# shichaoy/pop_up_slam

Measured on AMD Instinct MI355X. Metric: graph-solve iters/sec + final chi2, 1k-pose/5k-edge plane graph, higher is better.
Workload: dtype f64; 1 GPU; C2 synthetic corridor: 1000 SE3 poses, 200 planes, 5000 plane edges, 999 odometry edges (BASELINE.json configs[1], seed 42); jacobian_mode=numeric, total_lm_solves=805

## Files before the change

pop_up_slam_amd/csrc/pps_api.cpp:

```cpp
#include "pps_graph.h"

using namespace pps;
using namespace pps_impl;

namespace pps {
Switches read_switches() {
  auto on = [](const char* k) { return getenv(k) != nullptr; };
  auto num = [](const char* k, long long dflt) { const char* e = getenv(k); return e && *e ? atoll(e) : dflt; };
  Switches s;
  s.k1_thread_form = on("PPS_K1_THREAD_FORM");
  {
    long long plain = num("PPS_PLAIN_SCHEDULE", 0);
    if (on("PPS_PLAIN_SCHEDULE") && plain <= 0) plain = 15;
    s.no_preassemble = (plain & 1) != 0; s.no_solve_flow = (plain & 2) != 0; s.no_root_fuse = (plain & 4) != 0; s.split_expand = (plain & 8) != 0;
  }
  s.no_spec_lin = on("PPS_NO_SPEC_LIN");
  s.no_dual = on("PPS_NO_DUAL");
  s.no_strip = on("PPS_NO_STRIP");
  s.no_incremental = on("PPS_NO_INCREMENTAL");
  s.no_incr_compact = on("PPS_NO_INCR_COMPACT");
  s.verify_upload = on("PPS_DEBUG_VERIFY_UPLOAD");
  s.multi_levels = on("PPS_MULTI_LEVELS");
  s.multi_thread_form = on("PPS_MULTI_THREAD_FORM");
  s.debug_drop_flag = (int)num("PPS_DEBUG_DROP_FLAG", 0);
  if (on("PPS_DEBUG_DROP_FLAG") && s.debug_drop_flag < 1) s.debug_drop_flag = 1;
  s.trace = (int)num("PPS_TRACE", 0);
  if (on("PPS_TRACE") && s.trace < 1) s.trace = 1;
  {
    long long tm = num("PPS_TIMING", 0);
// ... 108 lines not shown
    std::vector<std::pair<std::string, double>> v(g->up_laps.begin(), g->up_laps.end());
    std::sort(v.begin(), v.end());
    for (auto& kv : v) fprintf(stderr, "[upload] %-34s %9.3f ms total\n", kv.first.c_str(), 1e3 * kv.second);
  }
  if (g->acache) analysis_cache_free(g->acache);
  if (g->dev_ready) {
    (void)hipSetDevice(g->props.device);
    (void)hipStreamSynchronize(g->stream);
    free_device(g);
    release_arenas(g);
    if (g->host_result) (void)hipHostFree(g->host_result);
    if (g->ev[0]) (void)hipEventDestroy(g->ev[0]);
    if (g->ev[1]) (void)hipEventDestroy(g->ev[1]);
    for (hipEvent_t e : g->k1_events) (void)hipEventDestroy(e);
    for (hipEvent_t e : g->fk_events) (void)hipEventDestroy(e);
    if (g->d_lms) (void)hipFree(g->d_lms);
    if (g->h_lms) (void)hipHostFree(g->h_lms);
    if (g->d_queries) (void)hipHostFree(g->d_queries);
    if (g->d_results) (void)hipHostFree(g->d_results);
    if (g->d_lm_planes) (void)hipFree(g->d_lm_planes);
    if (g->rp_pin) (void)hipHostFree(g->rp_pin);
    cov_release(g);
    (void)hipStreamDestroy(g->stream);
  }
  delete g;
  return PPS_OK;
}

int pps_get_props(const pps_graph* g, pps_props* out) {
  if (!g || !out) return PPS_EINVAL;
// ... 441 lines not shown
```

pop_up_slam_amd/csrc/pps_device.h:

```cpp
#pragma once

#include <hip/hip_runtime.h>

#include <cstdint>

#include "pps_cost.h"

namespace pps {

struct DevGraph {
  int n_pose = 0, n_plane = 0, pose_ld = 0, plane_ld = 0;
  double *pose_est = nullptr, *pose_lin = nullptr;
  double *plane_est = nullptr, *plane_lin = nullptr;
  int *pose_voff = nullptr, *plane_voff = nullptr;
  int n_obs = 0, n_odo = 0, n_pp = 0, n_lp = 0;
  int obs_ld = 0, odo_ld = 0, pp_ld = 0, lp_ld = 0;
  int *obs_pose = nullptr, *obs_plane = nullptr; double *obs_meas = nullptr, *obs_w = nullptr;
  int n_obs_fixed = 0; double* obs_ray = nullptr;
  int *odo_a = nullptr, *odo_b = nullptr;         double *odo_meas = nullptr, *odo_w = nullptr;
  int *pp_pose = nullptr;                          double *pp_meas = nullptr, *pp_w = nullptr;
  int *lp_plane = nullptr;                         double *lp_meas = nullptr, *lp_w = nullptr;
  double* J = nullptr;
  int64_t joff_obs = 0, joff_odo = 0, joff_pp = 0, joff_lp = 0;
  double* P = nullptr;
// ... 44 lines not shown
  int no_strip = 0;
  unsigned sw = 0;
  double step_ac[4] = {0, 0, 0, 0};
  double* gwork = nullptr;
  int64_t gwork_stride = 0;
};

constexpr double kStatusInternal = 64.0;
enum : unsigned { SW_K1_THREAD_FORM = 1u, SW_NO_SOLVE_FLOW = 2u, SW_NO_ROOT_FUSE = 4u, SW_DEBUG_DROP_FLAG = 8u, SW_DEBUG_DROP_XFLAG = 16u };
struct Switches {
  bool k1_thread_form = false;
  bool no_preassemble = false;
  bool no_solve_flow = false;
  bool no_root_fuse = false;
  bool split_expand = false;
  bool no_spec_lin = false;
  bool no_dual = false;
  bool no_strip = false;
  bool no_incremental = false;
  bool no_incr_compact = false;
  bool verify_upload = false;
  bool multi_levels = false, multi_thread_form = false;
  int debug_drop_flag = 0;
  int trace = 0;
  bool analysis_timing = false, upload_timing = false;
  int multi_timing = 0;
  int multi_split = 0;
  long long multi_thread_factors = 120000;
  unsigned dev_bits() const {
    return (k1_thread_form ? SW_K1_THREAD_FORM : 0u) | (no_solve_flow ? SW_NO_SOLVE_FLOW : 0u) | (no_root_fuse ? SW_NO_ROOT_FUSE : 0u) |
// ... 29 lines not shown
hipError_t step_constants(double ac[4]);
hipError_t launch_linearize(const DevGraph& d, int mode, bool at_estimate, hipStream_t st, const LinGuard* guard = nullptr, hipEvent_t ev0 = nullptr,
                            hipEvent_t ev1 = nullptr);
hipError_t launch_hblocks(const DevGraph& d, hipStream_t st, const LinGuard* guard = nullptr, bool products = true);
bool k1_lane_form(const DevGraph& d, int mode);
bool k1_products(const DevGraph& d, int mode);
hipError_t launch_factor_level(const DevGraph& d, int level_begin, int level_count, int level_max_front, double lambda,
                               hipStream_t st);
hipError_t launch_backsolve_level(const DevGraph& d, int level_begin, int level_count, hipStream_t st);
struct DualAlt {
  double *L, *U, *delta, *result_dev, *chi2_partials, *dn_partials;
  unsigned int* ticket;
  double lambda;
};
hipError_t launch_band_all(const DevGraph& d, const DualAlt* alt, int n_groups, int nwaves_factor, int nwaves_solve, int max_front, int max_panel,
                           int max_group_fronts, double lambda, int epoch, hipStream_t st, hipEvent_t ev0 = nullptr, hipEvent_t ev1 = nullptr);
int band_all_solve_waves(int max_panel, int max_group_fronts);
hipError_t launch_band_factor(const DevGraph& d, int grp_begin, int grp_count, int nwaves, int max_front, double lambda, hipStream_t st,
                              hipEvent_t ev0 = nullptr, hipEvent_t ev1 = nullptr, bool pre = false);
hipError_t launch_band_solve(const DevGraph& d, int grp_begin, int grp_count, int nwaves, int max_panel, int max_group_fronts, hipStream_t st,
                             const DualAlt* alt = nullptr);
hipError_t launch_band_factor_dual(const DevGraph& d, const DualAlt& alt, int grp_begin, int grp_count, int nwaves, int max_front, double lambda,
                                   hipStream_t st, hipEvent_t ev0 = nullptr, hipEvent_t ev1 = nullptr, bool pre = false);
bool band_root_fusable(const DevGraph& d, int grp_count, int max_front);
hipError_t launch_band_root(const DevGraph& d, const DualAlt* alt, int grp, int nwaves_factor, int nwaves_solve, int max_front, int max_panel,
                            int max_group_fronts, double lambda, hipStream_t st, hipEvent_t ev0 = nullptr, hipEvent_t ev1 = nullptr,
                            bool pre = false);
hipError_t launch_trial_dual(const DevGraph& d, const DualAlt& alt, const double* base_pose, const double* base_plane, double* out_pose0,
                             double* out_plane0, double* out_pose1, double* out_plane1, double* host_result0, double seq0, double* host_result1,
                             double seq1, hipStream_t st, int n_trials = 2);
hipError_t launch_trial_lin(const DevGraph& d, const DualAlt& alt, const SpecLin& sl, const double* base_pose, const double* base_plane, double* out_pose0,
                            double* out_plane0, double* out_pose1, double* out_plane1, double* host_result0, double seq0, double* host_result1,
// ... 93 lines not shown
```

pop_up_slam_amd/csrc/pps_graph.h:

```cpp
#pragma once
#include <hip/hip_runtime.h>

#include <algorithm>
#include <charconv>
#include <chrono>
#include <cmath>
#include <cstdio>
#include <cstdlib>
#include <cstring>
#include <mutex>
#include <new>
#include <string>
#include <unordered_map>
#include <vector>

#include "../../include/pps.h"
#include "pps_cov.h"
#include "pps_device.h"
#include "pps_geom.h"
#include "pps_lm.h"
#include "pps_popup_dev.h"
#include "pps_symbolic.h"

namespace pps_impl {
// ... 86 lines not shown
  bool pin_holds_est = false;
  std::unordered_map<std::string, double> up_laps;
  struct UpPatch { size_t off, len; bool exact8 = false; };
  std::vector<UpPatch> up_patches;
  char* patch_host = nullptr; size_t patch_cap = 0;
  size_t up_bytes_sent = 0, up_bytes_total = 0;
  double* host_result = nullptr;
  double seq = 0.0;
  double *spec_pose = nullptr, *spec_plane = nullptr, *spec_chi2_partials = nullptr, *spec_dn_partials = nullptr;
  unsigned int* spec_ticket = nullptr;
  double seq2 = 0.0;
  double *spec_L = nullptr, *spec_U = nullptr, *spec_delta = nullptr;
  double* spec_result = nullptr;
  double *spec_J = nullptr, *spec_P = nullptr, *spec_H = nullptr, *spec_Hf = nullptr;
  bool k3_all = false;
  int k3_nw_factor = 0, k3_nw_solve = 0, k3_max_front = 0, k3_max_panel = 0, k3_max_grp = 0, k3_epoch = 0;
  double *snap_pose = nullptr, *snap_plane = nullptr;
  int snap_version = -1, upload_version = 0;
  int k2t_version = -1;
  int profiling = 0;
  hipEvent_t ev[2] = {nullptr, nullptr};
  unsigned long long launches0 = 0;
  std::vector<char> k1_skip;
  std::vector<hipEvent_t> k1_events;
  std::vector<hipEvent_t> fk_events;
  int fk_used = 0;
  int k1_used = 0;
  float frames_invK[9] = {1, 0, 0, 0, 1, 0, 0, 0, 1};
  std::vector<int> fr_pose;
  std::vector<int> fr_seg_off{0};
  std::vector<float> fr_seg;
  std::vector<int> fr_item_frame, fr_item_plane, fr_item_fid;
  bool frames_dirty = true;
  std::vector<int> fr_slot, fr_pslot;
  long n_removals = 0, fr_cache_removals = -1;
  int fr_hint_version = -2; size_t fr_hint_cursor = 0, fr_hint_items = 0, fr_hint_frames = 0;
  int frames_version = -1;
  int *d_item_frame = nullptr, *d_item_plane = nullptr, *d_item_slot = nullptr, *d_frame_pose_slot = nullptr, *d_frame_seg_off = nullptr;
  float* d_fr_seg = nullptr;
  bool dev_meas_newer = false;
  int n_obs_fixed = 0;
// ... 219 lines not shown
```

pop_up_slam_amd/csrc/pps_k3.hip:

```cpp
#include <algorithm>
#include <atomic>
#include <cstdlib>

#include <hip/hip_ext.h>

#include "pps_kcommon.h"
#include "pps_regtile.h"
#include "pps_front_reg.h"

namespace pps {


constexpr int kLdsLimitBytes = 160 * 1024 - 1024;

int lds_front_limit() {
  int fa = 1;
  while ((size_t)(fa + 1) * ((fa + 1) | 1) * 8 <= (size_t)kLdsLimitBytes) fa++;
  return fa - 1;
}

template <bool USE_LDS>
__global__ __launch_bounds__(256) void k_front_factor(DevGraph d, int level_begin, double lambda) {
  extern __shared__ double lds[];
  const int s = d.level_fronts[level_begin + blockIdx.x];
// ... 417 lines not shown
  __builtin_amdgcn_wave_barrier();
}
struct XGroup { int* flag; int epoch; };
__device__ __forceinline__ void xg_post(const XGroup& x, int s) {
  __builtin_amdgcn_fence(__ATOMIC_RELEASE, "agent");
  if ((threadIdx.x & 63) == 0) __hip_atomic_store(x.flag + s, x.epoch, __ATOMIC_RELAXED, __HIP_MEMORY_SCOPE_AGENT);
}
__device__ __forceinline__ void xg_wait(const DevGraph& d, const XGroup& x, int s) {
  int spin = 0;
  while (__hip_atomic_load(x.flag + s, __ATOMIC_RELAXED, __HIP_MEMORY_SCOPE_AGENT) != x.epoch) {
    if (++spin >= (1 << 21)) { if ((threadIdx.x & 63) == 0) raise_status(&d.result_dev[2], kStatusInternal); break; }
    __builtin_amdgcn_s_sleep(2);
  }
  __builtin_amdgcn_fence(__ATOMIC_ACQUIRE, "agent");
}
template <bool XG = false>
__device__ __forceinline__ void front_extend_add(const DevGraph& d, int rec, int crv0, int lane, double* __restrict__ F, int tr, const XGroup* xg = nullptr) {
  const int cr0 = __builtin_amdgcn_readlane(rec, 5), nch = __builtin_amdgcn_readlane(rec, 6);
  for (int cb = 0; cb < nch; cb += 8) {
    const int crv = cb == 0 ? crv0 : ((lane < 8 * (nch - cb)) ? d.crec[(size_t)(cr0 + cb) * 8 + lane] : 0);
    auto child = [&](int cj, int& n, const double* __restrict__& Uc, const int* __restrict__& tgc) {
      n = __builtin_amdgcn_readlane(crv, 8 * cj);
      const long long uo = ((long long)__builtin_amdgcn_readlane(crv, 8 * cj + 2) << 32) | (unsigned int)__builtin_amdgcn_readlane(crv, 8 * cj + 1);
      const long long eo = ((long long)__builtin_amdgcn_readlane(crv, 8 * cj + 4) << 32) | (unsigned int)__builtin_amdgcn_readlane(crv, 8 * cj + 3);
      Uc = d.U + uo; tgc = d.ea_tgt + eo;
    };
    int cj = 0;
    for (; cj < 8 && cb + cj < nch; cj++) {
      int n; const double* Uc; const int* tgc;
      child(cj, n, Uc, tgc);
// ... 65 lines not shown
#ifndef PPS_NO_FMA
#pragma clang fp contract(fast)
#endif
    if (!SCALED) solve_pivot_scale(lk, dinv);
#define PPS_BS(U) case U: tj -= lk[U] * row_bcast_d<U>(tj); [[fallthrough]];
    switch (p < 16 ? p - 1 : 15) {
      PPS_BS(15) PPS_BS(14) PPS_BS(13) PPS_BS(12) PPS_BS(11) PPS_BS(10) PPS_BS(9) PPS_BS(8)
      PPS_BS(7) PPS_BS(6) PPS_BS(5) PPS_BS(4) PPS_BS(3) PPS_BS(2)
      case 1: tj -= lk[1] * row_bcast_d<1>(tj); [[fallthrough]];
      default: break;
    }
#undef PPS_BS
    tj *= dinv;
}

template <bool GROUP = true, bool TR = false, bool XG = false>
__device__ __forceinline__ void wave_front_solve(const DevGraph& d, int rec, double* __restrict__ W, double* __restrict__ X, int slot, int* flow = nullptr, const XGroup* xg = nullptr) {
  const int lane = threadIdx.x & 63;
  const int s = __builtin_amdgcn_readlane(rec, 0);
  (void)s;
  if (TR) PPS_TR(0);
  const int p = __builtin_amdgcn_readlane(rec, 1), b = __builtin_amdgcn_readlane(rec, 2), f = p + b;
  const double* __restrict__ Lp = d.L + (((long long)__builtin_amdgcn_readlane(rec, 10) << 32) | (unsigned int)__builtin_amdgcn_readlane(rec, 9));
  const int pslot = GROUP ? __builtin_amdgcn_readlane(rec, 14) : -1;
  const int* __restrict__ ix = b == 0 ? d.frec : (pslot >= 0 ? d.cmap + __builtin_amdgcn_readlane(rec, 15) : d.bidx + __builtin_amdgcn_readlane(rec, 8));
  double* xb = W;
  double* PL = W + kBandMaxRows;
  const int ix0r = ix[lane < b ? lane : 0], ix1r = ix[lane + 64 < b ? lane + 64 : 0];
  const int pix = d.pidx[__builtin_amdgcn_readlane(rec, 7) + (lane < p ? lane : 0)];
  const int n = (f + 1) * p;
  double tj = 0.0, dinv = 0.0;
// ... 9 lines not shown
    double lbv[12];
#pragma unroll
    for (int u = 0; u < 12; u++) { const int i = part + 4 * u; lbv[u] = LB[(i < b ? i : blast) * p]; }
#pragma unroll
    for (int u = 0; u < 16; u++) { const double l = Lp[(u < p ? u : p - 1) * p + lc]; lk[u] = lane < u ? l : 0.0; }
    const double dg = Lp[lc * p + lc], yr = Lp[f * p + jc];
    const int ix0 = lane < b ? ix0r : 0, ix1 = lane + 64 < b ? ix1r : 0;
    double g0 = 0.0, g1 = 0.0;
    const int xpar = XG ? __builtin_amdgcn_readlane(rec, 13) : -1;
    if (pslot < 0 && xpar < 0) { g0 = d.delta[ix0]; g1 = d.delta[ix1]; }
    if (flow) { dinv = 1.0 / dg; solve_pivot_scale(lk, dinv); }
    if (pslot >= 0) {
      if (flow) flow_wait(d, flow, pslot);
      const double* __restrict__ Xp = X + (size_t)pslot * kBandMaxRows; g0 = Xp[ix0]; g1 = Xp[ix1];
    } else if (XG && xpar >= 0) {
      xg_wait(d, *xg, xpar);
      g0 = d.delta[ix0]; g1 = d.delta[ix1];
    }
    if (TR) PPS_TR(1);
    if (lane < b) xb[lane] = g0;
    if (lane + 64 < b) xb[lane + 64] = g1;
    __builtin_amdgcn_wave_barrier();
    if (TR) PPS_TR(2);
    if (!flow) dinv = 1.0 / dg;
    double a[4] = {part == 0 ? yr : 0.0, 0.0, 0.0, 0.0};
#pragma unroll
    for (int u = 0; u < 12; u++) { const int i = part + 4 * u; const double x = i < b ? xb[i] : 0.0; a[u & 3] -= lbv[u] * x; }
    for (int i0 = 48; i0 < b; i0 += 48) {
#pragma unroll
      for (int u = 0; u < 12; u++) { const int i = i0 + part + 4 * u; lbv[u] = LB[(i < b ? i : blast) * p]; }
#pragma unroll
// ... 51 lines not shown
    if (pre32) {
      const int sh = p <= 16 ? 4 : 5, np = 64 >> sh;
      const int j = lane & ((1 << sh) - 1), part = lane >> sh;
      const int jc = j < p ? j : 0;
      const int blast = b > 0 ? b - 1 : 0;
#pragma unroll
      for (int u = 0; u < 12; u++) { const int i = part + np * u; lbq[u] = PL[(p + (i < b ? i : blast)) * p + jc]; }
      yq = PL[f * p + jc];
    }
  }
  if (pslot >= 0) {
    if (flow) flow_wait(d, flow, pslot);
    const double* __restrict__ Xp = X + (size_t)pslot * kBandMaxRows;
    g0 = Xp[ix0]; g1 = Xp[ix1];
  } else if (XG && xpar >= 0) {
    xg_wait(d, *xg, xpar);
    g0 = d.delta[ix0]; g1 = d.delta[ix1];
  }
  if (lane < b) xb[lane] = g0;
  if (lane + 64 < b) xb[lane + 64] = g1;
  __builtin_amdgcn_wave_barrier();
  if (TR) PPS_TR(2);
  {
#ifndef PPS_NO_FMA
#pragma clang fp contract(fast)
#endif
    if (!flow) {
#pragma unroll
      for (int u = 0; u < 16; u++) { const int k = k0 + u; const double l = PL[(k < p ? k : p - 1) * p + lc]; lk[u] = lane < k ? l : 0.0; }
      dinv = 1.0 / PL[lc * p + lc];
    }
// ... 35 lines not shown
    }
    solve_pivot_chain(p, lk, dinv, tj);
  }
  if (TR) PPS_TR(4);
  if (lane < p) d.delta[pix] = tj;
  if (TR) PPS_TR(5);
  if (!GROUP) return;
  double* __restrict__ Xs = X + (size_t)slot * kBandMaxRows;
  if (lane < p) Xs[lane] = tj;
  if (lane < b) Xs[p + lane] = g0;
  if (lane + 64 < b) Xs[p + lane + 64] = g1;
  if (flow) flow_post(d, flow, slot, pslot < 0);
  if (XG) { if (__builtin_amdgcn_readlane(rec, 6) > 0) xg_post(*xg, s); }
}

template <bool TR = false, bool XG = false>
__device__ __forceinline__ void body_band_solve_flow(const DevGraph& d, int g, int lds_doubles_per_wave, double* __restrict__ lds, int mg, const XGroup* xg = nullptr) {
  const int wave = uni(threadIdx.x >> 6), nw = blockDim.x >> 6;
  double* W = lds + (size_t)wave * lds_doubles_per_wave;
  double* X = lds + (size_t)nw * lds_doubles_per_wave;
  int* flow = reinterpret_cast<int*>(X + (size_t)mg * kBandMaxRows);
  const int2 span = reinterpret_cast<const int2*>(d.grp_span)[4 * (size_t)g];
  const int g0 = uni(span.x), gn = uni(span.y);
  const int i_first = g0 + gn - 1 - wave;
  int rec = i_first >= g0 ? d.frec[(size_t)i_first * 16 + (threadIdx.x & 15)] : 0;
  for (int q = threadIdx.x; q < gn; q += blockDim.x) flow[q] = 0;
  __syncthreads();
  for (int i = i_first; i >= g0; i -= nw) {
    wave_front_solve<true, TR, XG>(d, rec, W, X, i - g0, flow, xg);
    if (i - nw >= g0) rec = d.frec[(size_t)(i - nw) * 16 + (threadIdx.x & 15)];
  }
}
template <bool TR = false>
__device__ __forceinline__ void body_band_solve(const DevGraph& d, int g, int lds_doubles_per_wave, double* __restrict__ lds) {
  const int wave = uni(threadIdx.x >> 6), nw = blockDim.x >> 6;
  double* W = lds + (size_t)wave * lds_doubles_per_wave;
  double* X = lds + (size_t)nw * lds_doubles_per_wave;
  const int l0 = uni(d.grp_lvl_off[g]), l1 = uni(d.grp_lvl_off[g + 1]);
  int off[5], r4[4];
  {
    const int4 ga = reinterpret_cast<const int4*>(d.grp_span)[2 * (size_t)g], gb = reinterpret_cast<const int4*>(d.grp_span)[2 * (size_t)g + 1];
    off[0] = uni(ga.x); off[1] = uni(ga.w); off[2] = uni(gb.x); off[3] = uni(gb.y); off[4] = uni(gb.z);
  }
  const int g0 = off[0];
// ... 135 lines not shown
}

__global__ __launch_bounds__(512) void k_band_factor_all(DevGraph d, DualAlt alt, double lambda, int lds_doubles_per_wave, int epoch) {
  extern __shared__ double lds[];
  XGroup xg{d.k3_flag, epoch};
  if (blockIdx.y) { d.L = alt.L; d.U = alt.U; d.delta = alt.delta; d.result_dev = alt.result_dev; lambda = alt.lambda; xg.flag += d.n_fronts; }
  body_band_factor_pre<true>(d, blockIdx.x, lambda, lds_doubles_per_wave, lds, &xg);
}
__global__ __launch_bounds__(768) void k_band_solve_all(DevGraph d, DualAlt alt, int n_groups, int lds_doubles_per_wave, int mg, int epoch) {
  extern __shared__ double lds[];
  XGroup xg{d.k3_flag + 2 * d.n_fronts, epoch};
  if (blockIdx.y) { d.L = alt.L; d.U = alt.U; d.delta = alt.delta; d.result_dev = alt.result_dev; xg.flag += d.n_fronts; }
  body_band_solve_flow<false, true>(d, n_groups - 1 - (int)blockIdx.x, lds_doubles_per_wave, lds, mg, &xg);
}

__global__ __launch_bounds__(512) void k_band_factor_pre(DevGraph d, DualAlt alt, int grp_begin, double lambda, int lds_doubles_per_wave) {
  extern __shared__ double lds[];
  if (blockIdx.y) { d.L = alt.L; d.U = alt.U; d.delta = alt.delta; d.result_dev = alt.result_dev; lambda = alt.lambda; }
  body_band_factor_pre(d, grp_begin + blockIdx.x, lambda, lds_doubles_per_wave, lds);
}

__global__ __launch_bounds__(512) void k_band_factor_lean_trace(DevGraph d, DualAlt alt, int grp_begin, double lambda, int lds_doubles_per_wave) {
  extern __shared__ double lds[];
  body_band_factor<true, false, true>(d, grp_begin + blockIdx.x, lambda, lds_doubles_per_wave, lds);
}

__global__ __launch_bounds__(256) __attribute__((amdgpu_waves_per_eu(1, 1)))
void k_band_factor_r5(DevGraph d, DualAlt alt, int grp_begin, double lambda, int lds_doubles_per_wave) {
  extern __shared__ double lds[];
  if (blockIdx.y) { d.L = alt.L; d.U = alt.U; d.delta = alt.delta; d.result_dev = alt.result_dev; lambda = alt.lambda; }
// ... 9 lines not shown
    hipError_t e = hipFuncSetAttribute(reinterpret_cast<const void*>(&k_band_factor<false>), hipFuncAttributeMaxDynamicSharedMemorySize, kLdsLimitBytes);
    if (e == hipSuccess) e = hipFuncSetAttribute(reinterpret_cast<const void*>(&k_band_factor<true>), hipFuncAttributeMaxDynamicSharedMemorySize, kLdsLimitBytes);
    if (e == hipSuccess) e = hipFuncSetAttribute(reinterpret_cast<const void*>(&k_band_solve), hipFuncAttributeMaxDynamicSharedMemorySize, kLdsLimitBytes);
    if (e == hipSuccess) e = hipFuncSetAttribute(reinterpret_cast<const void*>(&k_band_solve_trace), hipFuncAttributeMaxDynamicSharedMemorySize, kLdsLimitBytes);
    if (e == hipSuccess) e = hipFuncSetAttribute(reinterpret_cast<const void*>(&k_band_solve_flow), hipFuncAttributeMaxDynamicSharedMemorySize, kLdsLimitBytes);
    if (e == hipSuccess) e = hipFuncSetAttribute(reinterpret_cast<const void*>(&k_band_factor_pre), hipFuncAttributeMaxDynamicSharedMemorySize, kLdsLimitBytes);
    if (e == hipSuccess) e = hipFuncSetAttribute(reinterpret_cast<const void*>(&k_band_solve_flow_trace), hipFuncAttributeMaxDynamicSharedMemorySize, kLdsLimitBytes);
    if (e == hipSuccess) e = hipFuncSetAttribute(reinterpret_cast<const void*>(&k_band_factor_r5), hipFuncAttributeMaxDynamicSharedMemorySize, kLdsLimitBytes);
    if (e == hipSuccess) e = hipFuncSetAttribute(reinterpret_cast<const void*>(&k_band_factor_lean_trace), hipFuncAttributeMaxDynamicSharedMemorySize, kLdsLimitBytes);
    if (e == hipSuccess) e = hipFuncSetAttribute(reinterpret_cast<const void*>(&k_band_root<false, false>), hipFuncAttributeMaxDynamicSharedMemorySize, kLdsLimitBytes);
    if (e == hipSuccess) e = hipFuncSetAttribute(reinterpret_cast<const void*>(&k_band_root<true, false>), hipFuncAttributeMaxDynamicSharedMemorySize, kLdsLimitBytes);
    if (e == hipSuccess) e = hipFuncSetAttribute(reinterpret_cast<const void*>(&k_band_root<false, true>), hipFuncAttributeMaxDynamicSharedMemorySize, kLdsLimitBytes);
    if (e == hipSuccess) e = hipFuncSetAttribute(reinterpret_cast<const void*>(&k_band_root<true, true>), hipFuncAttributeMaxDynamicSharedMemorySize, kLdsLimitBytes);
    if (e == hipSuccess) e = hipFuncSetAttribute(reinterpret_cast<const void*>(&k_band_factor_all), hipFuncAttributeMaxDynamicSharedMemorySize, kLdsLimitBytes);
    if (e == hipSuccess) e = hipFuncSetAttribute(reinterpret_cast<const void*>(&k_band_solve_all), hipFuncAttributeMaxDynamicSharedMemorySize, kLdsLimitBytes);
    if (e != hipSuccess) return e;
    g_band_attr_set[dev & 63] = true;
  }
  return hipSuccess;
}

static hipError_t launch_band_factor_impl(const DevGraph& d, const DualAlt& alt, int ny, int grp_begin, int grp_count, int nwaves, int max_front, double lambda,
                                          hipStream_t st, hipEvent_t ev0 = nullptr, hipEvent_t ev1 = nullptr, bool pre = false) {
  if (grp_count == 0) return hipSuccess;
  { const hipError_t e = ensure_band_attrs(); if (e != hipSuccess) return e; }
  const bool reg_only = max_front + 1 <= kRegRows && !(ny == 2 && d.trace != nullptr);
  const int per_wave = (int)(band_lds_bytes(max_front, reg_only) / sizeof(double));
  const size_t bytes = (size_t)per_wave * nwaves * sizeof(double);
  if (reg_only && d.trace != nullptr)
    PPS_LAUNCH(k_band_factor_lean_trace, dim3(grp_count, ny), dim3(64 * nwaves), bytes, st, d, alt, grp_begin, lambda, per_wave);
// ... 61 lines not shown
    const int want = nwaves_factor > (max_group_fronts < 8 ? max_group_fronts : 8) ? nwaves_factor : (max_group_fronts < 8 ? max_group_fronts : 8);
    if ((size_t)pws * want * sizeof(double) + flow_fixed <= (size_t)kLdsLimitBytes) nw = want; else flow = false;
  }
  const size_t bf = (size_t)pwf * nw * sizeof(double);
  const size_t bs = flow ? (size_t)pws * nw * sizeof(double) + flow_fixed : ((size_t)pws * nw + (size_t)max_group_fronts * kBandMaxRows) * sizeof(double);
  const size_t bytes = bf > bs ? bf : bs;
  const DualAlt a2 = alt ? *alt : DualAlt{};
  if (pre && flow) PPS_LAUNCH_EV(ev0, ev1, (k_band_root<true, true>), dim3(1, alt ? 2 : 1), dim3(64 * nw), bytes, st, d, a2, grp, lambda, pwf, pws, max_group_fronts);
  else if (pre) PPS_LAUNCH_EV(ev0, ev1, (k_band_root<true, false>), dim3(1, alt ? 2 : 1), dim3(64 * nw), bytes, st, d, a2, grp, lambda, pwf, pws, max_group_fronts);
  else if (flow) PPS_LAUNCH_EV(ev0, ev1, (k_band_root<false, true>), dim3(1, alt ? 2 : 1), dim3(64 * nw), bytes, st, d, a2, grp, lambda, pwf, pws, max_group_fronts);
  else PPS_LAUNCH_EV(ev0, ev1, (k_band_root<false, false>), dim3(1, alt ? 2 : 1), dim3(64 * nw), bytes, st, d, a2, grp, lambda, pwf, pws, max_group_fronts);
  return hipGetLastError();
}

hipError_t launch_band_all(const DevGraph& d, const DualAlt* alt, int n_groups, int nwaves_factor, int nwaves_solve, int max_front, int max_panel,
                           int max_group_fronts, double lambda, int epoch, hipStream_t st, hipEvent_t ev0, hipEvent_t ev1) {
  { const hipError_t e = ensure_band_attrs(); if (e != hipSuccess) return e; }
  const int pwf = (int)(band_lds_bytes(max_front, true) / sizeof(double)), pws = (int)(band_solve_lds_bytes(max_panel) / sizeof(double));
  const DualAlt a2 = alt ? *alt : DualAlt{};
  PPS_LAUNCH_EV(ev0, ev1, k_band_factor_all, dim3(n_groups, alt ? 2 : 1), dim3(64 * nwaves_factor), (size_t)pwf * nwaves_factor * sizeof(double), st, d, a2, lambda, pwf, epoch);
  const size_t fixed = ((size_t)max_group_fronts * kBandMaxRows + (size_t)(max_group_fronts + 1) / 2) * sizeof(double);
  PPS_LAUNCH(k_band_solve_all, dim3(n_groups, alt ? 2 : 1), dim3(64 * nwaves_solve), (size_t)pws * nwaves_solve * sizeof(double) + fixed, st, d, a2, n_groups, pws, max_group_fronts, epoch);
  return hipGetLastError();
}
int band_all_solve_waves(int max_panel, int max_group_fronts) {
  const size_t per_wave = band_solve_lds_bytes(max_panel);
  const size_t fixed = ((size_t)max_group_fronts * kBandMaxRows + (size_t)(max_group_fronts + 1) / 2) * sizeof(double);
  const size_t room = (size_t)kLdsLimitBytes > fixed ? ((size_t)kLdsLimitBytes - fixed) / per_wave : 0;
  return (int)std::min<size_t>(std::min<size_t>(12, (size_t)max_group_fronts), room);
}

__global__ __launch_bounds__(64) void k_front_solve(DevGraph d, int level_begin) {
  __shared__ double t[256];
  const int s = d.level_fronts[level_begin + blockIdx.x];
  const int p = d.f_p[s], b = d.f_b[s], f = p + b;
  const double* __restrict__ Lp = d.L + d.f_Loff[s];
  const int* __restrict__ bi = d.bidx + d.f_bidx_off[s];
// ... 340 lines not shown
```

pop_up_slam_amd/csrc/pps_solve.cpp:

```cpp
#include "pps_graph.h"

using namespace pps;
using namespace pps_impl;

namespace pps_impl {

struct PhaseTimer {
  pps_graph* g; double* acc; bool on;
  PhaseTimer(pps_graph* g_, double* a) : g(g_), acc(a), on(g_->profiling >= 2) { if (on) (void)hipEventRecord(g->ev[0], g->stream); }
  ~PhaseTimer() {
    if (!on) return;
    (void)hipEventRecord(g->ev[1], g->stream);
    (void)hipEventSynchronize(g->ev[1]);
    float ms = 0;
    (void)hipEventElapsedTime(&ms, g->ev[0], g->ev[1]);
    *acc += 1e-3 * ms;
  }
};

int do_linearize(pps_graph* g, const LinGuard* guard = nullptr) {
  if (g->profiling == 1) {
    if (g->k1_used + 2 > (int)g->k1_events.size()) {
      for (int k = 0; k < 2; k++) { hipEvent_t e; HIP_TRY(g, hipEventCreate(&e)); g->k1_events.push_back(e); }
    }
    g->k1_skip.resize(g->k1_events.size() / 2, 0);
    g->k1_skip[g->k1_used / 2] = 0;
    HIP_TRY(g, lin_launch(g, g->props.jacobian_mode, false, guard, g->k1_events[g->k1_used], g->k1_events[g->k1_used + 1]));
    g->k1_used += 2;
  } else
  { PhaseTimer t(g, &g->stats.t_linearize); HIP_TRY(g, lin_launch(g, g->props.jacobian_mode, false, guard)); }
  { PhaseTimer t(g, &g->stats.t_assemble); HIP_TRY(g, launch_hblocks(g->dev, g->stream, guard, k1_products(g->dev, g->props.jacobian_mode))); }
  if (!guard) g->stats.n_linearize++;
  return PPS_OK;
}

static int enqueue_factor_solve(pps_graph* g, const DevGraph& dv, const DualAlt* alt, double lambda, hipStream_t st_, bool events) {
  const Analysis& A = g->an;
  if (g->k3_all) {
    hipEvent_t e0 = nullptr, e1 = nullptr;
    if (events) {
      if (g->fk_used + 2 > (int)g->fk_events.size()) for (int k = 0; k < 2; k++) { hipEvent_t e; HIP_TRY(g, hipEventCreate(&e)); g->fk_events.push_back(e); }
      e0 = g->fk_events[g->fk_used]; e1 = g->fk_events[g->fk_used + 1]; g->fk_used += 2;
    }
    g->k3_epoch = g->k3_epoch >= (1 << 30) ? 1 : g->k3_epoch + 1;
    HIP_TRY(g, launch_band_all(dv, alt, A.n_groups, g->k3_nw_factor, g->k3_nw_solve, g->k3_max_front, g->k3_max_panel, g->k3_max_grp, lambda, g->k3_epoch, st_, e0, e1));
    return PPS_OK;
  }
  const int top = A.n_stages - 1;
  const bool fuse = top >= 0 && band_root_fusable(dv, A.stage_grp_off[top + 1] - A.stage_grp_off[top], A.stage_max_front[top]);
  for (int st = 0; st < A.n_stages; st++) {
    hipEvent_t e0 = nullptr, e1 = nullptr;
    if (events) {
      if (g->fk_used + 2 > (int)g->fk_events.size()) for (int k = 0; k < 2; k++) { hipEvent_t e; HIP_TRY(g, hipEventCreate(&e)); g->fk_events.push_back(e); }
      e0 = g->fk_events[g->fk_used]; e1 = g->fk_events[g->fk_used + 1]; g->fk_used += 2;
    }
    const int g0 = A.stage_grp_off[st], ng = A.stage_grp_off[st + 1] - g0;
    const bool pre = st < (int)g->stage_pre.size() && g->stage_pre[st] != 0;
    if (fuse && st == top)
      HIP_TRY(g, launch_band_root(dv, alt, g0, g->stage_nw_factor[st], g->stage_nw_solve[st], A.stage_max_front[st], g->stage_max_panel[st],
                                  g->stage_max_grp_fronts[st], lambda, st_, e0, e1, pre));
// ... 113 lines not shown
  return PPS_OK;
}

void resolve_k1_events(pps_graph* g) {
  for (int k = 0; k + 1 < g->k1_used; k += 2) {
    float ms = 0;
    if ((size_t)(k / 2) < g->k1_skip.size() && g->k1_skip[k / 2]) continue;
    if (hipEventElapsedTime(&ms, g->k1_events[k], g->k1_events[k + 1]) == hipSuccess) g->stats.t_linearize += 1e-3 * ms;
  }
  g->k1_used = 0;
  for (int k = 0; k + 1 < g->fk_used; k += 2) {
    float ms = 0;
    if (hipEventElapsedTime(&ms, g->fk_events[k], g->fk_events[k + 1]) == hipSuccess) g->stats.t_factor += 1e-3 * ms;
  }
  g->fk_used = 0;
}

static void reset_solve_stats(pps_graph* g) {
  pps_stats& s = g->stats;
  s.t_linearize = s.t_assemble = s.t_factor = s.t_backsolve = s.t_retract_chi2 = 0;
  s.n_linearize = s.n_factorize = 0;
  s.lm_iterations = s.lm_trials_accepted = s.lm_trials_rejected = s.lm_trials_notpd = 0;
  s.t_analysis = s.t_upload = 0;
  s.n_launches = 0;
  g->launches0 = launch_count();
}

void begin_solve(pps_graph* g) {
  reset_solve_stats(g);
  g->tr_lambda.clear(); g->tr_chi2.clear(); g->tr_acc.clear();
// ... 329 lines not shown
```

pop_up_slam_amd/csrc/pps_upload.cpp:

```cpp
#include "pps_graph.h"

using namespace pps;
using namespace pps_impl;

namespace pps_impl {

void free_device(pps_graph* g) {
  for (void* p : g->allocs) (void)hipFree(p);
  g->allocs.clear();
  for (pps_graph::Arena* a : {&g->up, &g->scr}) {
    const size_t want = (a == &g->up ? std::max(a->off, g->up_high) : a->off) + a->spill;
    if (a->spill > 0 || a->base == nullptr) {
      if (a->base) (void)hipFree(a->base);
      a->cap = std::max<size_t>(size_t(1) << 20, 2 * want);
      if (hipMalloc(reinterpret_cast<void**>(&a->base), a->cap) != hipSuccess) { a->base = nullptr; a->cap = 0; }
      if (a == &g->up) { g->up_slots.clear(); g->up_high = 0; g->up_unknown = true; }
    }
    a->off = 0; a->spill = 0;
  }
  g->up_cursor = 0; g->up_patches.clear();
  if (g->stage_cap < g->up.cap) {
    if (g->stage) (void)hipHostFree(g->stage);
    g->stage = nullptr; g->stage_cap = 0;
    if (hipHostMalloc(reinterpret_cast<void**>(&g->stage), g->up.cap, hipHostMallocDefault) == hipSuccess) g->stage_cap = g->up.cap;
// ... 286 lines not shown
      for (int st = 0; st < A.n_stages; st++) {
        bool ok = A.stage_grp_off[st + 1] > A.stage_grp_off[st] && A.stage_max_front[st] + 1 <= band_reg_rows();
        const int nw = g->stage_nw_factor[st];
        for (int gi = A.stage_grp_off[st]; ok && gi < A.stage_grp_off[st + 1]; gi++) {
          const int l0 = A.grp_lvl_off[gi], nl = A.grp_lvl_off[gi + 1] - l0;
          ok = nl >= 1 && nl <= 4;
          int upper = 0, c0 = 0;
          for (int k = 0; ok && k < nl; k++) {
            const int c = A.glvl_front_off[l0 + k + 1] - A.glvl_front_off[l0 + k];
            if (k == 0) c0 = c; else upper += c;
          }
          ok = ok && (c0 + upper <= nw || (nl >= 3 && c0 <= nw && upper <= nw));
        }
        g->stage_pre[st] = ok ? 1 : 0;
      }
    g->k3_all = false;
    if (g->use_band && A.n_stages >= 2 && g->sw.trace == 0 && !g->sw.no_preassemble && !g->sw.no_solve_flow && !g->sw.no_root_fuse && A.n_groups <= 100) {
      bool ok = true;
      int nwf = 1, mf = 0, mp = 1, mg = 1;
      for (int st = 0; st < A.n_stages; st++) {
        ok = ok && g->stage_pre[st] != 0 && A.stage_max_front[st] + 1 <= band_reg_rows();
        nwf = std::max(nwf, g->stage_nw_factor[st]); mf = std::max(mf, A.stage_max_front[st]);
        mp = std::max(mp, g->stage_max_panel[st]); mg = std::max(mg, g->stage_max_grp_fronts[st]);
      }
      const int nws = ok ? band_all_solve_waves(mp, mg) : 0;
      ok = ok && mg > 1 && nws >= std::min(8, mg) && band_lds_bytes(mf, true) * (size_t)nwf <= lds_budget;
      if (ok) { g->k3_all = true; g->k3_nw_factor = nwf; g->k3_nw_solve = nws; g->k3_max_front = mf; g->k3_max_panel = mp; g->k3_max_grp = mg; }
    }
  }
  if (!g->use_band && !g->use_dense && g->an.max_front > 4096)
    return fail(g, PPS_ENOMEM, "fronts too wide for this ordering (max front " + std::to_string(g->an.max_front) +
                               " scalars): the pose chain is not a good dissection backbone for this graph");
  if (g->sw.analysis_timing) fprintf(stderr, "[analysis] %-22s %8.3f ms\n", "total incl. api", 1e3 * (now_s() - t0));
  g->analyzed = true; g->analysis_stale = false;
  g->n_analyses++; g->grown_only = true;
  g->an_base_seq = g->an_seq; g->an_seq++;
  g->stats.n_fronts = g->an.n_fronts; g->stats.n_levels = g->an.n_levels; g->stats.max_front = g->an.max_front;
  g->stats.nnz_L = g->an.L_size;
  g->stats.t_analysis = now_s() - t0;
  return PPS_OK;
}

// ... 296 lines not shown
      r[0] = A.glvl_front_off[l0]; r[1] = A.glvl_front_off[l0 + nl] - r[0]; r[2] = nl;
      for (int k = 1; k <= 4; k++) r[2 + k] = A.glvl_front_off[l0 + std::min(k, nl)];
    }
    TRY(dev_upload(g, &d.grp_span, span));
  }
  TRY(dev_upload(g, &d.glvl_fronts, A.glvl_fronts));
  TRY(dev_upload(g, &d.frec, A.frec)); TRY(dev_upload(g, &d.crec, A.crec)); TRY(dev_upload(g, &d.srec, A.srec, 8 * kS));
  TRY(dev_upload(g, &d.obs_dir, A.obs_dir)); TRY(dev_upload(g, &d.nd_segs, A.nd_segs, (size_t)K.nd_segs)); d.n_nd_segs = (int)A.nd_segs.size();
  TRY(dev_upload(g, &d.cls_off, A.cls_off)); TRY(dev_upload(g, &d.cls_fronts, A.cls_fronts));
  if (g->use_dense) { TRY(dev_upload(g, &g->d_dw_asm, g->dw_asm)); TRY(dev_upload(g, &g->d_dw_pan, g->dw_pan)); TRY(dev_upload(g, &g->d_dw_trl, g->dw_trl)); }
  d.chi2_blocks = (d.n_obs + 255) / 256 + (d.n_odo + 255) / 256 + (d.n_pp + 255) / 256 + (d.n_lp + 255) / 256;
  TRY(dev_alloc(g, &d.chi2_partials, (size_t)std::max(1, d.chi2_blocks)));

  {
    const size_t n_dn = (size_t)(d.n_pose + d.n_plane + 255) / 256 + 1;
    const size_t flag_doubles = 2 * (size_t)std::max(1, A.n_fronts) + 1;
    double* zb = nullptr;
    TRY(dev_alloc(g, &zb, n_dn + 2 + 8 + 2 * delta_doubles + flag_doubles));
    zero_block = zb; zero_doubles = n_dn + 2 + 8 + 2 * delta_doubles + flag_doubles;
    d.k3_flag = reinterpret_cast<int*>(zb + n_dn + 2 + 8 + 2 * delta_doubles);
    g->k3_epoch = 0;
    d.delta = zb + n_dn + 10; g->spec_delta = d.delta + delta_doubles;
    d.dn_partials = zb;
    d.ticket = reinterpret_cast<unsigned int*>(zb + n_dn);
    g->spec_ticket = reinterpret_cast<unsigned int*>(zb + n_dn + 1);
    d.result_dev = zb + n_dn + 2; g->spec_result = zb + n_dn + 6;
    g->status_clean = true;
  }
  TRY(dev_alloc(g, &g->spec_pose, state_doubles + 1)); g->spec_plane = g->spec_pose + (size_t)7 * d.pose_ld;
  TRY(dev_alloc(g, &g->spec_chi2_partials, (size_t)std::max(1, d.chi2_blocks)));
  TRY(dev_alloc(g, &g->spec_dn_partials, (size_t)(d.n_pose + d.n_plane + 255) / 256 + 1));
// ... 52 lines not shown
```

Measured before the change: 17260 LM iters/s.

## Fuse band factor and backsolve into a single tree kernel with cross-block flags

Adds k_band_tree_all, which runs the per-group band factorization and the backsolve in one launch. Non-root blocks factor their group and post a group flag, the root block factors and then solves, and extra walk-only blocks spin-wait on the group flags before solving their subtree. This removes one kernel launch and the inter-kernel gap per LM solve. The cost is that blocks spin on flags at agent scope, which risks stalls if the blocks are not co-resident. Also adds backsolve timing events for the non-tree path.

Result: slower. 16490 LM iters/s (-4.4%).

```diff
diff --git a/pop_up_slam_amd/csrc/pps_api.cpp b/pop_up_slam_amd/csrc/pps_api.cpp
--- a/pop_up_slam_amd/csrc/pps_api.cpp
+++ b/pop_up_slam_amd/csrc/pps_api.cpp
@@ -11,8 +11,9 @@
   s.k1_thread_form = on("PPS_K1_THREAD_FORM");
   {
     long long plain = num("PPS_PLAIN_SCHEDULE", 0);
-    if (on("PPS_PLAIN_SCHEDULE") && plain <= 0) plain = 15;
+    if (on("PPS_PLAIN_SCHEDULE") && plain <= 0) plain = 31;
     s.no_preassemble = (plain & 1) != 0; s.no_solve_flow = (plain & 2) != 0; s.no_root_fuse = (plain & 4) != 0; s.split_expand = (plain & 8) != 0;
+    s.no_tree_fuse = (plain & 16) != 0;
   }
   s.no_spec_lin = on("PPS_NO_SPEC_LIN");
   s.no_dual = on("PPS_NO_DUAL");
@@ -151,6 +152,7 @@
     if (g->ev[1]) (void)hipEventDestroy(g->ev[1]);
     for (hipEvent_t e : g->k1_events) (void)hipEventDestroy(e);
     for (hipEvent_t e : g->fk_events) (void)hipEventDestroy(e);
+    for (hipEvent_t e : g->bk_events) (void)hipEventDestroy(e);
     if (g->d_lms) (void)hipFree(g->d_lms);
     if (g->h_lms) (void)hipHostFree(g->h_lms);
     if (g->d_queries) (void)hipHostFree(g->d_queries);
diff --git a/pop_up_slam_amd/csrc/pps_device.h b/pop_up_slam_amd/csrc/pps_device.h
--- a/pop_up_slam_amd/csrc/pps_device.h
+++ b/pop_up_slam_amd/csrc/pps_device.h
@@ -82,6 +82,7 @@
   bool no_solve_flow = false;
   bool no_root_fuse = false;
   bool split_expand = false;
+  bool no_tree_fuse = false;
   bool no_spec_lin = false;
   bool no_dual = false;
   bool no_strip = false;
@@ -141,8 +142,12 @@
   double lambda;
 };
 hipError_t launch_band_all(const DevGraph& d, const DualAlt* alt, int n_groups, int nwaves_factor, int nwaves_solve, int max_front, int max_panel,
-                           int max_group_fronts, double lambda, int epoch, hipStream_t st, hipEvent_t ev0 = nullptr, hipEvent_t ev1 = nullptr);
+                           int max_group_fronts, double lambda, int epoch, hipStream_t st, hipEvent_t ev0 = nullptr, hipEvent_t ev1 = nullptr,
+                           hipEvent_t ev2 = nullptr, hipEvent_t ev3 = nullptr);
 int band_all_solve_waves(int max_panel, int max_group_fronts);
+bool band_tree_fits(int nwaves_factor, int max_front, int max_panel, int max_group_fronts);
+hipError_t launch_band_tree(const DevGraph& d, const DualAlt* alt, int n_groups, int nwaves_factor, int max_front, int max_panel, int max_group_fronts,
+                            double lambda, int epoch, hipStream_t st);
 hipError_t launch_band_factor(const DevGraph& d, int grp_begin, int grp_count, int nwaves, int max_front, double lambda, hipStream_t st,
                               hipEvent_t ev0 = nullptr, hipEvent_t ev1 = nullptr, bool pre = false);
 hipError_t launch_band_solve(const DevGraph& d, int grp_begin, int grp_count, int nwaves, int max_panel, int max_group_fronts, hipStream_t st,
diff --git a/pop_up_slam_amd/csrc/pps_graph.h b/pop_up_slam_amd/csrc/pps_graph.h
--- a/pop_up_slam_amd/csrc/pps_graph.h
+++ b/pop_up_slam_amd/csrc/pps_graph.h
@@ -124,6 +124,7 @@
   double* spec_result = nullptr;
   double *spec_J = nullptr, *spec_P = nullptr, *spec_H = nullptr, *spec_Hf = nullptr;
   bool k3_all = false;
+  bool k3_tree = false;
   int k3_nw_factor = 0, k3_nw_solve = 0, k3_max_front = 0, k3_max_panel = 0, k3_max_grp = 0, k3_epoch = 0;
   double *snap_pose = nullptr, *snap_plane = nullptr;
   int snap_version = -1, upload_version = 0;
@@ -135,6 +136,8 @@
   std::vector<hipEvent_t> k1_events;
   std::vector<hipEvent_t> fk_events;
   int fk_used = 0;
+  std::vector<hipEvent_t> bk_events;
+  int bk_used = 0;
   int k1_used = 0;
   float frames_invK[9] = {1, 0, 0, 0, 1, 0, 0, 0, 1};
   std::vector<int> fr_pose;
diff --git a/pop_up_slam_amd/csrc/pps_k3.hip b/pop_up_slam_amd/csrc/pps_k3.hip
--- a/pop_up_slam_amd/csrc/pps_k3.hip
+++ b/pop_up_slam_amd/csrc/pps_k3.hip
@@ -455,6 +455,16 @@
   }
   __builtin_amdgcn_fence(__ATOMIC_ACQUIRE, "agent");
 }
+template <int NAP>
+__device__ __forceinline__ void xg_wait_early(const DevGraph& d, const XGroup& x, int s) {
+  int spin = 0;
+  while (__hip_atomic_load(x.flag + s, __ATOMIC_RELAXED, __HIP_MEMORY_SCOPE_AGENT) != x.epoch) {
+    if ((spin & 15) == 0 && __hip_atomic_load(&d.result_dev[2], __ATOMIC_RELAXED, __HIP_MEMORY_SCOPE_AGENT) >= kStatusInternal) break;
+    if (++spin >= (1 << 21)) { if ((threadIdx.x & 63) == 0) raise_status(&d.result_dev[2], kStatusInternal); break; }
+    __builtin_amdgcn_s_sleep(NAP);
+  }
+  __builtin_amdgcn_fence(__ATOMIC_ACQUIRE, "agent");
+}
 template <bool XG = false>
 __device__ __forceinline__ void front_extend_add(const DevGraph& d, int rec, int crv0, int lane, double* __restrict__ F, int tr, const XGroup* xg = nullptr) {
   const int cr0 = __builtin_amdgcn_readlane(rec, 5), nch = __builtin_amdgcn_readlane(rec, 6);
@@ -550,7 +560,7 @@
     tj *= dinv;
 }
 
-template <bool GROUP = true, bool TR = false, bool XG = false>
+template <bool GROUP = true, bool TR = false, bool XG = false, bool XE = false>
 __device__ __forceinline__ void wave_front_solve(const DevGraph& d, int rec, double* __restrict__ W, double* __restrict__ X, int slot, int* flow = nullptr, const XGroup* xg = nullptr) {
   const int lane = threadIdx.x & 63;
   const int s = __builtin_amdgcn_readlane(rec, 0);
@@ -590,7 +600,7 @@
       if (flow) flow_wait(d, flow, pslot);
       const double* __restrict__ Xp = X + (size_t)pslot * kBandMaxRows; g0 = Xp[ix0]; g1 = Xp[ix1];
     } else if (XG && xpar >= 0) {
-      xg_wait(d, *xg, xpar);
+      if (XE) xg_wait_early<2>(d, *xg, xpar); else xg_wait(d, *xg, xpar);
       g0 = d.delta[ix0]; g1 = d.delta[ix1];
     }
     if (TR) PPS_TR(1);
@@ -672,7 +682,7 @@
     const double* __restrict__ Xp = X + (size_t)pslot * kBandMaxRows;
     g0 = Xp[ix0]; g1 = Xp[ix1];
   } else if (XG && xpar >= 0) {
-    xg_wait(d, *xg, xpar);
+    if (XE) xg_wait_early<2>(d, *xg, xpar); else xg_wait(d, *xg, xpar);
     g0 = d.delta[ix0]; g1 = d.delta[ix1];
   }
   if (lane < b) xb[lane] = g0;
@@ -738,8 +748,9 @@
   if (XG) { if (__builtin_amdgcn_readlane(rec, 6) > 0) xg_post(*xg, s); }
 }
 
-template <bool TR = false, bool XG = false>
-__device__ __forceinline__ void body_band_solve_flow(const DevGraph& d, int g, int lds_doubles_per_wave, double* __restrict__ lds, int mg, const XGroup* xg = nullptr) {
+template <bool TR = false, bool XG = false, bool XE = false>
+__device__ __forceinline__ void body_band_solve_flow(const DevGraph& d, int g, int lds_doubles_per_wave, double* __restrict__ lds, int mg, const XGroup* xg = nullptr,
+                                                     const XGroup* gf = nullptr, bool gwait = false) {
   const int wave = uni(threadIdx.x >> 6), nw = blockDim.x >> 6;
   double* W = lds + (size_t)wave * lds_doubles_per_wave;
   double* X = lds + (size_t)nw * lds_doubles_per_wave;
@@ -749,9 +760,11 @@
   const int i_first = g0 + gn - 1 - wave;
   int rec = i_first >= g0 ? d.frec[(size_t)i_first * 16 + (threadIdx.x & 15)] : 0;
   for (int q = threadIdx.x; q < gn; q += blockDim.x) flow[q] = 0;
+  if (XE) { if (gwait && wave == 0) xg_wait_early<32>(d, *gf, g); }
   __syncthreads();
+  if (XE) { if (gwait) __builtin_amdgcn_fence(__ATOMIC_ACQUIRE, "agent"); }
   for (int i = i_first; i >= g0; i -= nw) {
-    wave_front_solve<true, TR, XG>(d, rec, W, X, i - g0, flow, xg);
+    wave_front_solve<true, TR, XG, XE>(d, rec, W, X, i - g0, flow, xg);
     if (i - nw >= g0) rec = d.frec[(size_t)(i - nw) * 16 + (threadIdx.x & 15)];
   }
 }
@@ -917,6 +930,26 @@
   body_band_solve_flow<false, true>(d, n_groups - 1 - (int)blockIdx.x, lds_doubles_per_wave, lds, mg, &xg);
 }
 
+__global__ __launch_bounds__(512) void k_band_tree_all(DevGraph d, DualAlt alt, int n_groups, double lambda, int per_wave_factor, int per_wave_solve, int mg, int epoch) {
+  extern __shared__ double lds[];
+  XGroup xf{d.k3_flag, epoch}, xs{d.k3_flag + 2 * d.n_fronts, epoch}, gf{d.k3_flag + 4 * d.n_fronts, epoch};
+  if (blockIdx.y) {
+    d.L = alt.L; d.U = alt.U; d.delta = alt.delta; d.result_dev = alt.result_dev; lambda = alt.lambda;
+    xf.flag += d.n_fronts; xs.flag += d.n_fronts; gf.flag += n_groups;
+  }
+  const int bx = (int)blockIdx.x;
+  const bool walk_only = bx >= n_groups;
+  if (!walk_only) {
+    body_band_factor_pre<true>(d, bx, lambda, per_wave_factor, lds, &xf);
+    if (bx != n_groups - 1) {
+      asm volatile("s_waitcnt vmcnt(0)\n\ts_barrier" ::: "memory");
+      if (threadIdx.x < 64) xg_post(gf, bx);
+      return;
+    }
+  }
+  body_band_solve_flow<false, true, true>(d, walk_only ? 2 * n_groups - 2 - bx : bx, per_wave_solve, lds, mg, &xs, &gf, walk_only);
+}
+
 __global__ __launch_bounds__(512) void k_band_factor_pre(DevGraph d, DualAlt alt, int grp_begin, double lambda, int lds_doubles_per_wave) {
   extern __shared__ double lds[];
   if (blockIdx.y) { d.L = alt.L; d.U = alt.U; d.delta = alt.delta; d.result_dev = alt.result_dev; lambda = alt.lambda; }
@@ -956,6 +989,7 @@
     if (e == hipSuccess) e = hipFuncSetAttribute(reinterpret_cast<const void*>(&k_band_root<true, true>), hipFuncAttributeMaxDynamicSharedMemorySize, kLdsLimitBytes);
     if (e == hipSuccess) e = hipFuncSetAttribute(reinterpret_cast<const void*>(&k_band_factor_all), hipFuncAttributeMaxDynamicSharedMemorySize, kLdsLimitBytes);
     if (e == hipSuccess) e = hipFuncSetAttribute(reinterpret_cast<const void*>(&k_band_solve_all), hipFuncAttributeMaxDynamicSharedMemorySize, kLdsLimitBytes);
+    if (e == hipSuccess) e = hipFuncSetAttribute(reinterpret_cast<const void*>(&k_band_tree_all), hipFuncAttributeMaxDynamicSharedMemorySize, kLdsLimitBytes);
     if (e != hipSuccess) return e;
     g_band_attr_set[dev & 63] = true;
   }
@@ -1047,13 +1081,30 @@
 }
 
 hipError_t launch_band_all(const DevGraph& d, const DualAlt* alt, int n_groups, int nwaves_factor, int nwaves_solve, int max_front, int max_panel,
-                           int max_group_fronts, double lambda, int epoch, hipStream_t st, hipEvent_t ev0, hipEvent_t ev1) {
+                           int max_group_fronts, double lambda, int epoch, hipStream_t st, hipEvent_t ev0, hipEvent_t ev1, hipEvent_t ev2, hipEvent_t ev3) {
   { const hipError_t e = ensure_band_attrs(); if (e != hipSuccess) return e; }
   const int pwf = (int)(band_lds_bytes(max_front, true) / sizeof(double)), pws = (int)(band_solve_lds_bytes(max_panel) / sizeof(double));
   const DualAlt a2 = alt ? *alt : DualAlt{};
   PPS_LAUNCH_EV(ev0, ev1, k_band_factor_all, dim3(n_groups, alt ? 2 : 1), dim3(64 * nwaves_factor), (size_t)pwf * nwaves_factor * sizeof(double), st, d, a2, lambda, pwf, epoch);
   const size_t fixed = ((size_t)max_group_fronts * kBandMaxRows + (size_t)(max_group_fronts + 1) / 2) * sizeof(double);
-  PPS_LAUNCH(k_band_solve_all, dim3(n_groups, alt ? 2 : 1), dim3(64 * nwaves_solve), (size_t)pws * nwaves_solve * sizeof(double) + fixed, st, d, a2, n_groups, pws, max_group_fronts, epoch);
+  PPS_LAUNCH_EV(ev2, ev3, k_band_solve_all, dim3(n_groups, alt ? 2 : 1), dim3(64 * nwaves_solve), (size_t)pws * nwaves_solve * sizeof(double) + fixed, st, d, a2, n_groups, pws, max_group_fronts, epoch);
+  return hipGetLastError();
+}
+static size_t band_tree_lds_bytes(int nw, int max_front, int max_panel, int max_group_fronts) {
+  const size_t fixed = ((size_t)max_group_fronts * kBandMaxRows + (size_t)(max_group_fronts + 1) / 2) * sizeof(double);
+  return std::max<size_t>(band_lds_bytes(max_front, true) * (size_t)nw, band_solve_lds_bytes(max_panel) * (size_t)nw + fixed);
+}
+bool band_tree_fits(int nwaves_factor, int max_front, int max_panel, int max_group_fronts) {
+  return max_group_fronts <= 8 && nwaves_factor >= max_group_fronts && nwaves_factor <= 8 &&
+         band_tree_lds_bytes(nwaves_factor, max_front, max_panel, max_group_fronts) <= (size_t)kLdsLimitBytes;
+}
+hipError_t launch_band_tree(const DevGraph& d, const DualAlt* alt, int n_groups, int nwaves_factor, int max_front, int max_panel, int max_group_fronts,
+                            double lambda, int epoch, hipStream_t st) {
+  { const hipError_t e = ensure_band_attrs(); if (e != hipSuccess) return e; }
+  const int pwf = (int)(band_lds_bytes(max_front, true) / sizeof(double)), pws = (int)(band_solve_lds_bytes(max_panel) / sizeof(double));
+  const DualAlt a2 = alt ? *alt : DualAlt{};
+  PPS_LAUNCH(k_band_tree_all, dim3(2 * n_groups - 1, alt ? 2 : 1), dim3(64 * nwaves_factor), band_tree_lds_bytes(nwaves_factor, max_front, max_panel, max_group_fronts), st, d, a2,
+             n_groups, lambda, pwf, pws, max_group_fronts, epoch);
   return hipGetLastError();
 }
 int band_all_solve_waves(int max_panel, int max_group_fronts) {
diff --git a/pop_up_slam_amd/csrc/pps_solve.cpp b/pop_up_slam_amd/csrc/pps_solve.cpp
--- a/pop_up_slam_amd/csrc/pps_solve.cpp
+++ b/pop_up_slam_amd/csrc/pps_solve.cpp
@@ -37,13 +37,19 @@
 static int enqueue_factor_solve(pps_graph* g, const DevGraph& dv, const DualAlt* alt, double lambda, hipStream_t st_, bool events) {
   const Analysis& A = g->an;
   if (g->k3_all) {
-    hipEvent_t e0 = nullptr, e1 = nullptr;
+    g->k3_epoch = g->k3_epoch >= (1 << 30) ? 1 : g->k3_epoch + 1;
+    if (g->k3_tree && g->profiling == 0) {
+      HIP_TRY(g, launch_band_tree(dv, alt, A.n_groups, g->k3_nw_factor, g->k3_max_front, g->k3_max_panel, g->k3_max_grp, lambda, g->k3_epoch, st_));
+      return PPS_OK;
+    }
+    hipEvent_t e0 = nullptr, e1 = nullptr, e2 = nullptr, e3 = nullptr;
     if (events) {
       if (g->fk_used + 2 > (int)g->fk_events.size()) for (int k = 0; k < 2; k++) { hipEvent_t e; HIP_TRY(g, hipEventCreate(&e)); g->fk_events.push_back(e); }
       e0 = g->fk_events[g->fk_used]; e1 = g->fk_events[g->fk_used + 1]; g->fk_used += 2;
-    }
-    g->k3_epoch = g->k3_epoch >= (1 << 30) ? 1 : g->k3_epoch + 1;
-    HIP_TRY(g, launch_band_all(dv, alt, A.n_groups, g->k3_nw_factor, g->k3_nw_solve, g->k3_max_front, g->k3_max_panel, g->k3_max_grp, lambda, g->k3_epoch, st_, e0, e1));
+      if (g->bk_used + 2 > (int)g->bk_events.size()) for (int k = 0; k < 2; k++) { hipEvent_t e; HIP_TRY(g, hipEventCreate(&e)); g->bk_events.push_back(e); }
+      e2 = g->bk_events[g->bk_used]; e3 = g->bk_events[g->bk_used + 1]; g->bk_used += 2;
+    }
+    HIP_TRY(g, launch_band_all(dv, alt, A.n_groups, g->k3_nw_factor, g->k3_nw_solve, g->k3_max_front, g->k3_max_panel, g->k3_max_grp, lambda, g->k3_epoch, st_, e0, e1, e2, e3));
     return PPS_OK;
   }
   const int top = A.n_stages - 1;
@@ -187,6 +193,11 @@
     if (hipEventElapsedTime(&ms, g->fk_events[k], g->fk_events[k + 1]) == hipSuccess) g->stats.t_factor += 1e-3 * ms;
   }
   g->fk_used = 0;
+  for (int k = 0; k + 1 < g->bk_used; k += 2) {
+    float ms = 0;
+    if (hipEventElapsedTime(&ms, g->bk_events[k], g->bk_events[k + 1]) == hipSuccess) g->stats.t_backsolve += 1e-3 * ms;
+  }
+  g->bk_used = 0;
 }
 
 static void reset_solve_stats(pps_graph* g) {
diff --git a/pop_up_slam_amd/csrc/pps_upload.cpp b/pop_up_slam_amd/csrc/pps_upload.cpp
--- a/pop_up_slam_amd/csrc/pps_upload.cpp
+++ b/pop_up_slam_amd/csrc/pps_upload.cpp
@@ -324,7 +324,7 @@
         }
         g->stage_pre[st] = ok ? 1 : 0;
       }
-    g->k3_all = false;
+    g->k3_all = false; g->k3_tree = false;
     if (g->use_band && A.n_stages >= 2 && g->sw.trace == 0 && !g->sw.no_preassemble && !g->sw.no_solve_flow && !g->sw.no_root_fuse && A.n_groups <= 100) {
       bool ok = true;
       int nwf = 1, mf = 0, mp = 1, mg = 1;
@@ -336,6 +336,8 @@
       const int nws = ok ? band_all_solve_waves(mp, mg) : 0;
       ok = ok && mg > 1 && nws >= std::min(8, mg) && band_lds_bytes(mf, true) * (size_t)nwf <= lds_budget;
       if (ok) { g->k3_all = true; g->k3_nw_factor = nwf; g->k3_nw_solve = nws; g->k3_max_front = mf; g->k3_max_panel = mp; g->k3_max_grp = mg; }
+      const int top = A.n_stages - 1;
+      g->k3_tree = ok && !g->sw.no_tree_fuse && A.stage_grp_off[top + 1] - A.stage_grp_off[top] == 1 && band_tree_fits(nwf, mf, mp, mg);
     }
   }
   if (!g->use_band && !g->use_dense && g->an.max_front > 4096)
@@ -662,7 +664,7 @@
 
   {
     const size_t n_dn = (size_t)(d.n_pose + d.n_plane + 255) / 256 + 1;
-    const size_t flag_doubles = 2 * (size_t)std::max(1, A.n_fronts) + 1;
+    const size_t flag_doubles = 2 * (size_t)std::max(1, A.n_fronts) + (size_t)std::max(1, A.n_groups) + 1;
     double* zb = nullptr;
     TRY(dev_alloc(g, &zb, n_dn + 2 + 8 + 2 * delta_doubles + flag_doubles));
     zero_block = zb; zero_doubles = n_dn + 2 + 8 + 2 * delta_doubles + flag_doubles;
```
